# bobhansky/WhittedStyle_Raytracer

Hardware: NVIDIA B200
Metric: Mrays/s (all ray types), out/water_bunny_tex.txt + shadow soft @ 3840x2160 (higher is better)
Workload: dtype f32

## Files before the change

### whittedstyle_raytracer_b200/csrc/cuda/bvh_build.cuh

```cuda
#pragma once
#include <cooperative_groups.h>
#include <cub/device/device_radix_sort.cuh>

#include <cfloat>

#include "ploc_bvh.h"
#include "shaft_cull.h"
#include "wide_bvh.h"
#include "../../../include/wrt_scene.h"

namespace wrt {

#define WRT_PLOC_THREADS 256

enum BuildState { BS_ALLOC = 0, BS_ROOT = 1, BS_DEPTH = 2, BS_PASSES = 3, BS_ERROR = 4, BS_LEAVES = 5, BS_TOTAL = 8 };

struct BuildBuffers {
    PlocTree tree;
    unsigned long long* keys[2];
    int* vals[2];
    int* cl[2];
    int* nn;
    int* blk;
    int* state;
// ... 180 lines not shown
        if (oct & 1) { t = lo.x; lo.x = hi.x; hi.x = t; }
        if (oct & 2) { t = lo.y; lo.y = hi.y; hi.y = t; }
        if (oct & 4) { t = lo.z; lo.z = hi.z; hi.z = t; }
        dst[2 * ((size_t)oct * n_nodes + i)] = lo;
        dst[2 * ((size_t)oct * n_nodes + i) + 1] = hi;
    }
}

__global__ void __launch_bounds__(256) k_wide4_copies(const float4* __restrict__ onodes, int n_nodes, float4* dst) {
    const int pairs = n_nodes / 2;
    const long long total = 8ll * pairs;
    for (long long g = blockIdx.x * (long long)blockDim.x + threadIdx.x; g < total; g += (long long)gridDim.x * blockDim.x) {
        const int oct = (int)(g / pairs);
        const int c = 2 * (int)(g - (long long)oct * pairs);
        if (c == 0) continue;
        float4 out[8];
        wrt_wide4_node(onodes + 2 * (size_t)oct * n_nodes, c, oct, out);
        float4* d = dst + WRT_WIDE_FLOAT4_PER_RECORD * ((size_t)oct * n_nodes + c);
#pragma unroll
        for (int i = 0; i < 8; i++) d[i] = out[i];
    }
}

__global__ void __launch_bounds__(256) k_pack_prims(int n_prims, const float* __restrict__ prim_geom, const unsigned* __restrict__ prim_flags,
                                                    const int* __restrict__ prim_material, const int* __restrict__ prim_texture,
                                                    const int* __restrict__ prim_normalmap, const int* __restrict__ prim_object,
                                                    const float* __restrict__ prim_normals, const float* __restrict__ prim_uv,
                                                    const float* __restrict__ materials, int n_materials, int n_textures, int n_normalmaps,
                                                    float4* geom, float4* attr, int4* ids, float4* tri_aux, int* flags_out) {
    int bad = 0;
    float slack = 0.f;
    for (int p = blockIdx.x * blockDim.x + threadIdx.x; p < n_prims; p += gridDim.x * blockDim.x) {
        const float* g = prim_geom + 12 * (size_t)p;
        const int mat = prim_material[p];
        const unsigned flags = prim_flags[p];
// ... 40 lines not shown
```

### whittedstyle_raytracer_b200/csrc/cuda/dev_traverse.cuh

```cuda
#pragma once
#include "dev_math.cuh"
#include "prune_rule.h"
#include "wide_bvh.h"
#include "shadow_assoc.h"
#include "../../../include/wrt_scene.h"

namespace wrt {

#define WRT_INLINE_LIGHTS 4

struct DevScene {
    const float4* nodes;
    const float4* fnodes;
    const float4* onodes;
    const float4* ronodes;
    const float4* wnodes;
    const float4* dnodes;
    const float4* geom;
    const float4* prim_box;
    const float4* tri_aux;
    const WrtPathCode* path_codes;
    const float4* attr;
    const int4*   ids;
    const int*    object_prim;
// ... 161 lines not shown
        asm volatile("prefetch.global.L1 [%0];" ::"l"(nodes + 2 * far_link));
#endif
        cur = right_first ? linkR : linkL;
        return true;
    }
    if (hl) { cur = linkL; return true; }
    if (hr) { cur = linkR; return true; }
    if (st.empty()) return false;
    cur = st.pop();
    return true;
}

#ifndef WRT_WIDE4
#define WRT_WIDE4 1
#endif
template <bool NEAR_FIRST, class LeafFn>
__device__ __forceinline__ bool traverse_step4(const float4* __restrict__ wnodes, const Ray& r, Stack& st, int& cur,
                                               const float& limit, LeafFn&& leaf) {
    const float4* n = wnodes + WRT_WIDE_FLOAT4_PER_RECORD * (size_t)cur;
    float4 a0, a1, b0, b1, c0, c1, d0, d1;
    ldg8(n, a0, a1);
    ldg8(n + 2, b0, b1);
    ldg8(n + 4, c0, c1);
    ldg8(n + 6, d0, d1);
    float t0, t1, t2, t3;
    bool h0 = slab_presorted(a0, a1, r, t0), h1 = slab_presorted(b0, b1, r, t1);
    bool h2 = slab_presorted(c0, c1, r, t2), h3 = slab_presorted(d0, d1, r, t3);
    int l0 = __float_as_int(a0.w), l1 = __float_as_int(b0.w), l2 = __float_as_int(c0.w), l3 = __float_as_int(d0.w);
    h0 = h0 && !(t0 > limit); h1 = h1 && !(t1 > limit); h2 = h2 && !(t2 > limit); h3 = h3 && !(t3 > limit);
    unsigned leaves = (h0 && l0 < 0 ? 1u : 0u) | (h1 && l1 < 0 ? 2u : 0u) | (h2 && l2 < 0 ? 4u : 0u) | (h3 && l3 < 0 ? 8u : 0u);
    while (leaves) {
        const unsigned j = __ffs(leaves) - 1;
        leaves &= leaves - 1;
        const int lk = j == 0 ? l0 : (j == 1 ? l1 : (j == 2 ? l2 : l3));
        const float tj = j == 0 ? t0 : (j == 1 ? t1 : (j == 2 ? t2 : t3));
        if (!(tj > limit)) leaf(~lk);
    }
    const float inf = INFINITY;
    float k0 = (h0 && l0 >= 0 && !(t0 > limit)) ? t0 : inf, k1 = (h1 && l1 >= 0 && !(t1 > limit)) ? t1 : inf;
    float k2 = (h2 && l2 >= 0 && !(t2 > limit)) ? t2 : inf, k3 = (h3 && l3 >= 0 && !(t3 > limit)) ? t3 : inf;
    if (NEAR_FIRST) {
#define WRT_CSWAP(ka, la, kb, lb) { const bool sw = kb < ka; const float kt = sw ? ka : kb; ka = sw ? kb : ka; kb = kt; const int lt = sw ? la : lb; la = sw ? lb : la; lb = lt; }
        WRT_CSWAP(k0, l0, k1, l1) WRT_CSWAP(k2, l2, k3, l3) WRT_CSWAP(k0, l0, k2, l2) WRT_CSWAP(k1, l1, k3, l3) WRT_CSWAP(k1, l1, k2, l2)
// ... 14 lines not shown
        if (nxt >= 0) { cur = nxt; return true; }
    }
    if (st.empty()) return false;
    cur = st.pop();
    return true;
}

#ifndef WRT_LEAF_DEFER
#define WRT_LEAF_DEFER 2
#endif
#ifndef WRT_LEAF_DEFER_SIMPLE
#define WRT_LEAF_DEFER_SIMPLE 1
#endif
#define WRT_NO_LINK (-2147483647 - 1)
template <bool NEAR_FIRST, class LeafFn>
__device__ __forceinline__ bool traverse_step4_defer(const float4* __restrict__ wnodes, const Ray& r, Stack& st, int& cur,
                                                     const float& limit, LeafFn&& leaf) {
    const float inf = INFINITY;
    int pend = WRT_NO_LINK;
    float tp = -inf;
    if (cur < 0) {
        pend = cur;
        cur = WRT_NO_LINK;
        if (!st.empty()) {
            const int nx = st.pop();
            if (nx >= 0) cur = nx; else ++st.sp;
        }
    }
    if (cur >= 0) {
        const float4* n = wnodes + WRT_WIDE_FLOAT4_PER_RECORD * (size_t)cur;
        float4 a0, a1, b0, b1, c0, c1, d0, d1;
        ldg8(n, a0, a1);
        ldg8(n + 2, b0, b1);
        ldg8(n + 4, c0, c1);
        ldg8(n + 6, d0, d1);
        float t0, t1, t2, t3;
        const bool h0 = slab_presorted(a0, a1, r, t0), h1 = slab_presorted(b0, b1, r, t1);
        const bool h2 = slab_presorted(c0, c1, r, t2), h3 = slab_presorted(d0, d1, r, t3);
        int l0 = __float_as_int(a0.w), l1 = __float_as_int(b0.w), l2 = __float_as_int(c0.w), l3 = __float_as_int(d0.w);
        float k0 = (h0 && !(t0 > limit)) ? t0 : inf, k1 = (h1 && !(t1 > limit)) ? t1 : inf;
        float k2 = (h2 && !(t2 > limit)) ? t2 : inf, k3 = (h3 && !(t3 > limit)) ? t3 : inf;
#define WRT_CSWAP(ka, la, kb, lb) { const bool sw = kb < ka; const float kt = sw ? ka : kb; ka = sw ? kb : ka; kb = kt; const int lt = sw ? la : lb; la = sw ? lb : la; lb = lt; }
        if (NEAR_FIRST) { WRT_CSWAP(k0, l0, k1, l1) WRT_CSWAP(k2, l2, k3, l3) WRT_CSWAP(k0, l0, k2, l2) WRT_CSWAP(k1, l1, k3, l3) WRT_CSWAP(k1, l1, k2, l2) }
#undef WRT_CSWAP
#if WRT_LEAF_DEFER_SIMPLE
        if (NEAR_FIRST) {
            const bool tk = (k0 < inf) && (l0 < 0) && (pend == WRT_NO_LINK);
            if (tk) { pend = l0; tp = k0; }
            const float kc = tk ? k1 : k0;
            const int lc = tk ? l1 : l0;
            cur = kc < inf ? lc : WRT_NO_LINK;
            if (k3 < inf) st.push(l3);
            if (k2 < inf) st.push(l2);
            if (!tk && k1 < inf) st.push(l1);
// ... 39 lines not shown
        limit = FLT_MAX; prune_scale = prune;
    }
    __device__ __forceinline__ void set_ray(const DevScene& s, const Ray& r, float prune_cfg) {
        const float o[3] = {r.o.x, r.o.y, r.o.z}, inv[3] = {r.inv.x, r.inv.y, r.inv.z};
        prune_scale = prune_cfg >= 0.f ? wrt_prune_ray_scale(o, inv, s.prune_slack) : -1.f;
    }
    __device__ __forceinline__ void leaf(const DevScene& s, const Ray& r, int p) {
        PrimHit h; float oma; unsigned fl;
        if (prim_test(s, p, r, h, oma, fl)) {
            if (h.t < best.t || (h.t == best.t && p < best.prim)) {
                best.t = h.t; best.prim = p; best.u = h.u; best.v = h.v;
                if (prune_scale >= 0.f) limit = wrt_prune_limit(h.t, prune_scale);
            }
        }
    }
    __device__ __forceinline__ bool begin(const DevScene& s, const float4* nodes, int root, const Ray& r, int& cur) {
        float te;
        float4 lo = ldg4(nodes + 2 * root), hi = ldg4(nodes + 2 * root + 1);
        if (!slab(lo, hi, r, te)) return false;
        int link = __float_as_int(lo.w);
        if (link < 0) { leaf(s, r, ~link); return false; }
        cur = link;
        return true;
    }
};

__device__ __forceinline__ Closest closest_hit(const DevScene& s, const float4* nodes, int root, const Ray& r, Stack& st,
                                               float prune_rel) {
    ClosestState cs;
    cs.reset(prune_rel);
// ... 44 lines not shown
        int k = i;
        while (k > 0 && prim[idx[k - 1]] > key) { idx[k] = idx[k - 1]; --k; }
        idx[k] = i;
    }
    for (int i = 0; i < n; i++) fs[i] = fac[idx[i]];
    return wrt_tree_product(n, idx, fs, code);
}

__device__ __forceinline__ float shadow_value(const DevScene& s, const ShadowAcc& acc) {
    return acc.needs_tree(s.path_codes) ? shadow_tree_value(acc.prim, acc.fac, acc.code, acc.n) : acc.res;
}

__device__ __forceinline__ void shadow_leaf(const DevScene& s, const Ray& r, float dis, int p, ShadowAcc& acc) {
    PrimHit h; float oma; unsigned fl;
    if (prim_test(s, p, r, h, oma, fl) && h.t < dis && !(fl & WRT_PRIM_LIGHT)) acc.add(p, oma, s.path_codes);
}

__device__ __forceinline__ float shadow_product(const DevScene& s, const float4* nodes, const Ray& r, float dis, Stack& st) {
    ShadowAcc acc;
    acc.reset();
    if (s.n_nodes == 0) return acc.res;
    float te;
    float4 lo = ldg4(nodes), hi = ldg4(nodes + 1);
    if (!slab(lo, hi, r, te)) return acc.res;
    int cur = __float_as_int(lo.w);
    if (cur < 0) { shadow_leaf(s, r, dis, ~cur, acc); return acc.res; }
    st.sp = 0;
    const float never = INFINITY;
    while (acc.res != 0.f && traverse_step<false>(nodes, r, st, cur, never, [&](int p) { shadow_leaf(s, r, dis, p, acc); })) {}
    return shadow_value(s, acc);
// ... 175 lines not shown
```

### whittedstyle_raytracer_b200/csrc/cuda/kernels.cuh

```cuda
#pragma once
#include <cooperative_groups.h>

#include "dev_shade.cuh"
#include "shaft_cull.h"
#include "../../../include/wrt_rng.h"
#include "../../../include/wrt_tiles.h"

#ifdef WRT_MIN_BLOCKS
#define WRT_TRACE_BOUNDS __launch_bounds__(128, WRT_MIN_BLOCKS)
#else
#define WRT_TRACE_BOUNDS __launch_bounds__(128)
#endif
#ifndef WRT_TRACE_DEEP_STEPS
#define WRT_TRACE_DEEP_STEPS 8
#endif
namespace wrt {

#ifdef WRT_DEBUG_BOUNDS
__device__ unsigned g_wrt_bounds_line = 0;
__device__ __forceinline__ bool wrt_bounds_ok(bool ok, unsigned line) {
    if (!ok) atomicCAS(&g_wrt_bounds_line, 0u, line);
    return ok;
}
#define WRT_IN_BOUNDS(idx, cap) wrt_bounds_ok((unsigned long long)(idx) < (unsigned long long)(cap), (unsigned)__LINE__)
// ... 291 lines not shown
        if (ref_tree) prune = -1.f;
        const size_t oct_off = (size_t)ray_octant(r.d) * 2 * (size_t)s.n_nodes;
        nodes = (ref_tree ? s.ronodes : s.onodes) + oct_off;
        cs.set_ray(s, r, prune);
        float te;
        float4 lo = ldg4(nodes), hi = ldg4(nodes + 1);
        if (!slab_presorted(lo, hi, r, te)) return false;
        cur = __float_as_int(lo.w);
        if (cur < 0) { cs.leaf(s, r, ~cur); return false; }
        wide = WRT_WIDE4 && !LEVEL0 && !ref_tree;
        if (wide) nodes = s.wnodes + (WRT_WIDE_FLOAT4_PER_RECORD / 2) * oct_off;
        return true;
    }
    __device__ __forceinline__ bool step(int& cur, Stack& st) {
#if WRT_LEAF_DEFER
        if (WRT_WIDE4 && !LEVEL0 && wide) return traverse_step4_defer<true>(nodes, r, st, cur, cs.limit, [&](int p) { cs.leaf(s, r, p); });
#else
        if (WRT_WIDE4 && !LEVEL0 && wide) return traverse_step4<true>(nodes, r, st, cur, cs.limit, [&](int p) { cs.leaf(s, r, p); });
#endif
        return traverse_step<true, true>(nodes, r, st, cur, cs.limit, [&](int p) { cs.leaf(s, r, p); });
    }
    __device__ __forceinline__ bool finish(int&, Stack&) {
        if (WRT_IN_BOUNDS(idx, fb.cap0 > fb.capd ? fb.cap0 : fb.capd))
            fb.hit[idx] = make_float4(cs.best.t, __int_as_float(cs.best.prim), cs.best.u, cs.best.v);
        return false;
    }
};

template <bool LEVEL0>
__global__ void WRT_TRACE_BOUNDS k_trace_closest(const __grid_constant__ DevScene s, const __grid_constant__ FrameBuffers fb,
                                                 const __grid_constant__ PrimaryGen pg, int level, unsigned n0, int work_slot,
                                                 float prune_rel, int refill) {
    extern __shared__ int smem[];
// ... 67 lines not shown
        const size_t oct_off = (size_t)ray_octant(raydir) * 2 * (size_t)s.n_nodes;
        nodes = (ref_tree ? s.ronodes : s.onodes) + oct_off;
        float te;
        float4 lo = ldg4(nodes), hi = ldg4(nodes + 1);
        if (!slab_presorted(lo, hi, r, te)) return false;
        cur = __float_as_int(lo.w);
        if (cur < 0) { shadow_leaf(s, r, dis, ~cur, acc); return false; }
        wide = WRT_WIDE4 && !ref_tree;
        if (wide) nodes = s.wnodes + (WRT_WIDE_FLOAT4_PER_RECORD / 2) * oct_off;
        return true;
    }
    __device__ __forceinline__ bool step(int& cur, Stack& st) {
        const float never = INFINITY;
        bool more;
#if WRT_LEAF_DEFER >= 2
        if (WRT_WIDE4 && wide) more = traverse_step4_defer<false>(nodes, r, st, cur, never, [&](int p) { shadow_leaf(s, r, dis, p, acc); });
#else
        if (WRT_WIDE4 && wide) more = traverse_step4<false>(nodes, r, st, cur, never, [&](int p) { shadow_leaf(s, r, dis, p, acc); });
#endif
        else more = traverse_step<false, true>(nodes, r, st, cur, never, [&](int p) { shadow_leaf(s, r, dis, p, acc); });
        return more && acc.res != 0.f;
    }
    __device__ __forceinline__ bool finish(int&, Stack&) {
        const float v = shadow_value(s, acc);
        if (WRT_IN_BOUNDS(out, (size_t)fb.n_node_cap * s.n_lights)) fb.coeff[out] = v;
        return false;
    }
};

__global__ void WRT_TRACE_BOUNDS k_shadow_hard(const __grid_constant__ DevScene s, const __grid_constant__ FrameBuffers fb, int q, int work_slot, int refill,
                                               int literal) {
    extern __shared__ int smem[];
    Stack st;
// ... 217 lines not shown
                    if (rc == 1) active = true;
                    else pend = rc;
                }
                head += need < avail ? need : avail;
                __syncwarp();
            }
            if (!__any_sync(0xffffffffu, active)) {
                if (drained && head == tail && !__any_sync(0xffffffffu, pend != -2)) break;
                continue;
            }
        }
#pragma unroll 1
        for (int it = 0; it < 4; it++) {
            if (active) {
#if WRT_WIDE4
                const int rc = wrt_shaft_walk_step4(&sh, &w, st.base, st.stride, stack_rows, mine, WRT_LIST_CAP);
#else
                const int rc = wrt_shaft_walk_step(&sh, &w, st.base, st.stride, stack_rows, mine, WRT_LIST_CAP);
#endif
                if (rc != 1) { active = false; pend = rc < 0 ? -1 : w.n; }
            }
        }
    }
    n_empty = __reduce_add_sync(0xffffffffu, n_empty);
    if (lane == 0 && n_empty) atomicAdd(fb.counters + C_NEMPTY, n_empty);
}
#else
__global__ void __launch_bounds__(128, WRT_LISTS_MIN_BLOCKS) k_soft_lists(const __grid_constant__ DevScene s, const __grid_constant__ FrameBuffers fb, int q,
                                                        int work_slot, int stack_rows, SoftListBuffers lb) {
    extern __shared__ int smem[];
    Stack st;
// ... 118 lines not shown
#endif
                        }
                        if (rc == 1) active = true;
                        else pend = rc;
                    }
                }
                if (!__any_sync(0xffffffffu, active)) {
                    if (next >= chunk && !__any_sync(0xffffffffu, pend != -2)) break;
                    continue;
                }
            }
#pragma unroll 1
            for (int it = 0; it < 4; it++) {
                if (active) {
#if WRT_WIDE4
                    const int rc = wrt_shaft_walk_step4(&sh, &w, st.base, st.stride, stack_rows, mine, WRT_LIST_CAP);
#else
                    const int rc = wrt_shaft_walk_step(&sh, &w, st.base, st.stride, stack_rows, mine, WRT_LIST_CAP);
#endif
                    if (rc != 1) { active = false; pend = rc < 0 ? -1 : w.n; }
                }
            }
        }
        __syncwarp();
    }
    n_empty = __reduce_add_sync(0xffffffffu, n_empty);
    if (lane == 0 && n_empty) atomicAdd(fb.counters + C_NEMPTY, n_empty);
}

#endif

// ... 525 lines not shown
```

### whittedstyle_raytracer_b200/csrc/cuda/shaft_cull.h

```cpp
#ifndef WRT_SHAFT_CULL_H
#define WRT_SHAFT_CULL_H

#include <math.h>

#include "wide_bvh.h"

#ifdef __CUDACC__
#define WRT_SHAFT_HD __host__ __device__ __forceinline__
#else
#include <vector_types.h>
#define WRT_SHAFT_HD static inline
#endif

#if defined(__CUDA_ARCH__)
#define WRT_SHAFT_LD4(p) __ldg(p)
#define WRT_SHAFT_LD8(p, a, b) wrt::ldg8(p, a, b)
#else
#define WRT_SHAFT_LD4(p) (*(p))
#define WRT_SHAFT_LD8(p, a, b) do { (a) = (p)[0]; (b) = (p)[1]; } while (0)
#endif

#define WRT_SHAFT_STACK 48
#define WRT_SHAFT_PAD_REL 1e-5f

// ... 58 lines not shown
    float ly = fminf(ay * sh->ilo[1], ay * sh->ihi[1]), uy = fmaxf(by * sh->ilo[1], by * sh->ihi[1]);
    float lz = fminf(az * sh->ilo[2], az * sh->ihi[2]), uz = fmaxf(bz * sh->ilo[2], bz * sh->ihi[2]);
    if (!(sh->use & 1)) { lx = -INFINITY; ux = INFINITY; }
    if (!(sh->use & 2)) { ly = -INFINITY; uy = INFINITY; }
    if (!(sh->use & 4)) { lz = -INFINITY; uz = INFINITY; }
    float lb = fmaxf(lx, fmaxf(ly, lz)), ub = fminf(ux, fminf(uy, uz));
    return lb <= ub && ub >= 0.f;
}

WRT_SHAFT_HD bool wrt_shaft_may_hit_lb(const WrtShaft* sh, const float4 nearp, const float4 farp, float* lb_out) {
    float ax = nearp.x - sh->o[0], ay = nearp.y - sh->o[1], az = nearp.z - sh->o[2];
    float bx = farp.x - sh->o[0], by = farp.y - sh->o[1], bz = farp.z - sh->o[2];
    float lx = fminf(ax * sh->ilo[0], ax * sh->ihi[0]), ux = fmaxf(bx * sh->ilo[0], bx * sh->ihi[0]);
    float ly = fminf(ay * sh->ilo[1], ay * sh->ihi[1]), uy = fmaxf(by * sh->ilo[1], by * sh->ihi[1]);
    float lz = fminf(az * sh->ilo[2], az * sh->ihi[2]), uz = fmaxf(bz * sh->ilo[2], bz * sh->ihi[2]);
    if (!(sh->use & 1)) { lx = -INFINITY; ux = INFINITY; }
    if (!(sh->use & 2)) { ly = -INFINITY; uy = INFINITY; }
    if (!(sh->use & 4)) { lz = -INFINITY; uz = INFINITY; }
    float lb = fmaxf(lx, fmaxf(ly, lz)), ub = fminf(ux, fminf(uy, uz));
    *lb_out = lb;
    return lb <= ub && ub >= 0.f;
}

typedef struct WrtShaftWalk {
    const float4* nodes;
    int cur, sp, n;
} WrtShaftWalk;

WRT_SHAFT_HD int wrt_shaft_walk_begin(const float4* onodes, int n_nodes, const WrtShaft* sh, WrtShaftWalk* w) {
    w->sp = 0; w->n = 0; w->cur = 0; w->nodes = onodes;
// ... 73 lines not shown
        w.f = r0.w; const int linkR = w.i;
        if ((hl && linkL < 0) || (hr && linkR < 0)) return false;
        if (hl && hr) {
            if (sp == WRT_SHAFT_STACK) return false;
            stack[sp++] = linkR;
            cur = linkL;
        } else if (hl) cur = linkL;
        else if (hr) cur = linkR;
        else {
            if (sp == 0) return true;
            cur = stack[--sp];
        }
    }
}

WRT_SHAFT_HD int wrt_shaft_walk_begin4(const float4* onodes, const float4* wnodes, int n_nodes, const WrtShaft* sh, WrtShaftWalk* w) {
    w->sp = 0; w->n = 0; w->cur = 0; w->nodes = wnodes;
    if (n_nodes <= 0) return 0;
    union { float f; int i; } u;
    u.f = WRT_SHAFT_LD4(onodes + (size_t)sh->octant * 2 * (size_t)n_nodes).w;
    w->cur = u.i;
    w->nodes = wnodes + WRT_WIDE_FLOAT4_PER_RECORD * (size_t)sh->octant * (size_t)n_nodes;
    return w->cur < 0 ? -1 : 1;
}

#ifndef WRT_SHAFT_STEP_BRANCHFREE
#define WRT_SHAFT_STEP_BRANCHFREE 1
#endif
#define WRT_SHAFT_CSWAP(ka, la, kb, lb) { const bool sw_ = (kb) < (ka); const float kt_ = sw_ ? (ka) : (kb); (ka) = sw_ ? (kb) : (ka); (kb) = kt_; \
                                          const int lt_ = sw_ ? (la) : (lb); (la) = sw_ ? (lb) : (la); (lb) = lt_; }

WRT_SHAFT_HD int wrt_shaft_walk_step4(const WrtShaft* sh, WrtShaftWalk* w, int* stack, int stack_stride, int stack_cap,
                                      int* out, int out_cap) {
    const float4* nd = w->nodes + WRT_WIDE_FLOAT4_PER_RECORD * (size_t)w->cur;
    float4 a0, a1, b0, b1, c0, c1, d0, d1;
    WRT_SHAFT_LD8(nd, a0, a1);
    WRT_SHAFT_LD8(nd + 2, b0, b1);
    WRT_SHAFT_LD8(nd + 4, c0, c1);
    WRT_SHAFT_LD8(nd + 6, d0, d1);
    float k0, k1, k2, k3;
    const bool h0 = wrt_shaft_may_hit_lb(sh, a0, a1, &k0), h1 = wrt_shaft_may_hit_lb(sh, b0, b1, &k1);
    const bool h2 = wrt_shaft_may_hit_lb(sh, c0, c1, &k2), h3 = wrt_shaft_may_hit_lb(sh, d0, d1, &k3);
    const float inf = INFINITY;
    if (!h0) k0 = inf;
    if (!h1) k1 = inf;
    if (!h2) k2 = inf;
    if (!h3) k3 = inf;
    union { float f; int i; } u;
    u.f = a0.w; int l0 = u.i;
    u.f = b0.w; int l1 = u.i;
    u.f = c0.w; int l2 = u.i;
    u.f = d0.w; int l3 = u.i;
    WRT_SHAFT_CSWAP(k0, l0, k1, l1) WRT_SHAFT_CSWAP(k2, l2, k3, l3) WRT_SHAFT_CSWAP(k0, l0, k2, l2)
    WRT_SHAFT_CSWAP(k1, l1, k3, l3) WRT_SHAFT_CSWAP(k1, l1, k2, l2)
    int n = w->n;
#if WRT_SHAFT_STEP_BRANCHFREE
    if (n + 4 > out_cap || w->sp + 3 > stack_cap) return -1;
    {
        const bool e0 = k0 < inf && l0 < 0, e1 = k1 < inf && l1 < 0, e2 = k2 < inf && l2 < 0, e3 = k3 < inf && l3 < 0;
        if (e0) out[n] = ~l0;
        n += e0 ? 1 : 0;
        if (e1) out[n] = ~l1;
        n += e1 ? 1 : 0;
        if (e2) out[n] = ~l2;
        n += e2 ? 1 : 0;
        if (e3) out[n] = ~l3;
        n += e3 ? 1 : 0;
// ... 24 lines not shown
    int next = -1;
    if (k3 < inf && l3 >= 0) next = l3;
    if (k2 < inf && l2 >= 0) { if (next >= 0) { if (w->sp == stack_cap) return -1; stack[w->sp * stack_stride] = next; ++w->sp; } next = l2; }
    if (k1 < inf && l1 >= 0) { if (next >= 0) { if (w->sp == stack_cap) return -1; stack[w->sp * stack_stride] = next; ++w->sp; } next = l1; }
    if (k0 < inf && l0 >= 0) { if (next >= 0) { if (w->sp == stack_cap) return -1; stack[w->sp * stack_stride] = next; ++w->sp; } next = l0; }
    if (next >= 0) { w->cur = next; return 1; }
    if (w->sp == 0) return 0;
    --w->sp;
    w->cur = stack[w->sp * stack_stride];
    return 1;
}

WRT_SHAFT_HD int wrt_shaft_candidates4(const float4* onodes, const float4* wnodes, int n_nodes, const WrtShaft* sh, int* stack,
                                       int stack_stride, int stack_cap, int* out, int out_cap) {
    WrtShaftWalk w;
    int rc = wrt_shaft_walk_begin4(onodes, wnodes, n_nodes, sh, &w);
    if (rc <= 0) return rc;
    while ((rc = wrt_shaft_walk_step4(sh, &w, stack, stack_stride, stack_cap, out, out_cap)) == 1) {}
    return rc < 0 ? -1 : w.n;
}

WRT_SHAFT_HD bool wrt_shaft_is_empty4(const float4* onodes, const float4* wnodes, int n_nodes, const float o[3], const float tri[9]) {
    if (n_nodes <= 0) return true;
    WrtShaft sh;
    if (!wrt_shaft_make(o, tri, &sh)) return false;
    union { float f; int i; } u;
    u.f = WRT_SHAFT_LD4(onodes + (size_t)sh.octant * 2 * (size_t)n_nodes).w;
    int cur = u.i;
    if (cur < 0) return false;
    const float4* nodes = wnodes + WRT_WIDE_FLOAT4_PER_RECORD * (size_t)sh.octant * (size_t)n_nodes;
    int stack[WRT_SHAFT_STACK];
    int sp = 0;
    while (true) {
        const float4* nd = nodes + WRT_WIDE_FLOAT4_PER_RECORD * (size_t)cur;
        float4 a0, a1, b0, b1, c0, c1, d0, d1;
        WRT_SHAFT_LD8(nd, a0, a1);
        WRT_SHAFT_LD8(nd + 2, b0, b1);
        WRT_SHAFT_LD8(nd + 4, c0, c1);
        WRT_SHAFT_LD8(nd + 6, d0, d1);
        const bool h0 = wrt_shaft_may_hit(&sh, a0, a1), h1 = wrt_shaft_may_hit(&sh, b0, b1);
        const bool h2 = wrt_shaft_may_hit(&sh, c0, c1), h3 = wrt_shaft_may_hit(&sh, d0, d1);
        u.f = a0.w; const int l0 = u.i;
        u.f = b0.w; const int l1 = u.i;
        u.f = c0.w; const int l2 = u.i;
        u.f = d0.w; const int l3 = u.i;
        if ((h0 && l0 < 0) || (h1 && l1 < 0) || (h2 && l2 < 0) || (h3 && l3 < 0)) return false;
        int next = -1;
        if (h3) next = l3;
        if (h2) { if (next >= 0) { if (sp == WRT_SHAFT_STACK) return false; stack[sp++] = next; } next = l2; }
        if (h1) { if (next >= 0) { if (sp == WRT_SHAFT_STACK) return false; stack[sp++] = next; } next = l1; }
        if (h0) { if (next >= 0) { if (sp == WRT_SHAFT_STACK) return false; stack[sp++] = next; } next = l0; }
        if (next >= 0) { cur = next; continue; }
        if (sp == 0) return true;
        cur = stack[--sp];
    }
}

typedef struct WrtShaftPyramid {
    float o[3];
    float D[4][3];
// ... 115 lines not shown
```

### whittedstyle_raytracer_b200/csrc/cuda/wide_bvh.h

```cpp
#ifndef WRT_WIDE_BVH_H
#define WRT_WIDE_BVH_H

#include <float.h>

#ifdef __CUDACC__
#define WRT_WIDE_HD __host__ __device__ __forceinline__
#else
#include <vector_types.h>
#define WRT_WIDE_HD static inline
#endif

#define WRT_WIDE_FLOAT4_PER_RECORD 4

WRT_WIDE_HD void wrt_wide4_node(const float4* src, int c, int oct, float4* out) {
    union { float f; int i; unsigned u; } w;
    for (int k = 0; k < 2; k++) {
        const float4 lo = src[2 * (size_t)(c + k)], hi = src[2 * (size_t)(c + k) + 1];
        w.f = lo.w;
        if (w.i >= 0) {
            const float4* ch = src + 2 * (size_t)w.i;
            out[4 * k + 0] = ch[0]; out[4 * k + 1] = ch[1];
            out[4 * k + 2] = ch[2]; out[4 * k + 3] = ch[3];
        } else {
            out[4 * k + 0] = lo; out[4 * k + 1] = hi;
            float4 e0, e1;
            e0.x = (oct & 1) ? -FLT_MAX : FLT_MAX; e1.x = -e0.x;
            e0.y = (oct & 2) ? -FLT_MAX : FLT_MAX; e1.y = -e0.y;
            e0.z = (oct & 4) ? -FLT_MAX : FLT_MAX; e1.z = -e0.z;
            w.u = 0x80000000u;
            e0.w = w.f; e1.w = 0.f;
            out[4 * k + 2] = e0; out[4 * k + 3] = e1;
        }
    }
}

#endif
```

### whittedstyle_raytracer_b200/csrc/cuda/wrt_cuda.cu

```cuda
#include <algorithm>
#include <cstdio>
#include <chrono>
#include <cstdlib>
#include <cstring>
#include <condition_variable>
#include <functional>
#include <mutex>
#include <string>
#include <thread>
#include <vector>

#include <cuda_runtime.h>

#include "../../../include/wrt_cuda.h"
#include "fast_bvh.hpp"
#include "kernels.cuh"
#include "bvh_build.cuh"

namespace {

thread_local std::string g_err;

int fail(const std::string& msg) {
    g_err = msg;
// ... 760 lines not shown
    ds.object_prim = (const int*)dptr(7);
    ds.lights = (const WrtLight*)dptr(11);
    ds.textures = (const WrtTexture*)dptr(12);
    ds.normalmaps = (const WrtTexture*)dptr(13);
    ds.texels = (const float*)dptr(14);
    ds.path_codes = parts[15].bytes ? (const WrtPathCode*)dptr(15) : nullptr;

    float4 *geom = nullptr, *attr = nullptr, *mats = nullptr, *pbox = nullptr, *taux = nullptr, *fnodes = nullptr, *dnodes = nullptr, *onodes = nullptr, *ronodes = nullptr, *wnodes = nullptr;
    int4* ids = nullptr;
    int* d_flags = nullptr;
    if (dev_alloc(c, (size_t)np * 48, (void**)&geom) || dev_alloc(c, (size_t)np * 64, (void**)&attr) || dev_alloc(c, (size_t)np * 16, (void**)&ids) ||
        dev_alloc(c, (size_t)s->n_materials * 48, (void**)&mats) || dev_alloc(c, (size_t)np * 32, (void**)&pbox) ||
        dev_alloc(c, (size_t)np * 16, (void**)&taux) ||
        dev_alloc(c, (size_t)nn * 32, (void**)&fnodes) || dev_alloc(c, (size_t)nn * 32, (void**)&dnodes) ||
        dev_alloc(c, (size_t)nn * 32 * 8, (void**)&onodes) || dev_alloc(c, (size_t)nn * 32 * 8, (void**)&ronodes) ||
        dev_alloc(c, (size_t)nn * 64 * 8, (void**)&wnodes) ||
        dev_alloc(c, (wrt::BS_TOTAL + 16) * sizeof(int), (void**)&d_flags))
        return 1;
    int* d_state = d_flags + 8;
    float* d_bounds = (float*)(d_flags + 8 + wrt::BS_TOTAL);
    CK(cudaMemsetAsync(d_flags, 0, (wrt::BS_TOTAL + 8) * sizeof(int), st));
    {
        const float init[8] = {FLT_MAX, FLT_MAX, FLT_MAX, -FLT_MAX, -FLT_MAX, -FLT_MAX, 0.f, 0.f};
        memcpy(c->h_counters + wrt::C_TOTAL + 32, init, sizeof init);
        CK(cudaMemcpyAsync(d_bounds, c->h_counters + wrt::C_TOTAL + 32, sizeof init, cudaMemcpyHostToDevice, st));
    }
    const int wide = c->num_sms * 4;
    if (np > 0) {
        ++c->launches;
        wrt::k_pack_prims<<<std::min(wide, (np + 255) / 256), 256, 0, st>>>(
            np, (const float*)dptr(1), (const unsigned*)dptr(2), (const int*)dptr(3), (const int*)dptr(4), (const int*)dptr(5),
// ... 749 lines not shown
```

Baseline: 7137.

## Compress wide BVH4 nodes to quantized 32-byte records with mirrored-ray traversal

Replaces the 64-byte four-child wide node (full float AABBs per child) with a 32-byte record: a per-node origin, per-axis power-of-two scale exponents, and 8-bit quantized child bounds, built with directed rounding so the boxes stay conservative. Traversal mirrors the ray into the positive octant and decodes the quantized bounds. Leaf hits are then confirmed against the exact primitive box, and the shaft-culling walk applies the same mirroring with an exact leaf check. The aim is to halve node memory traffic and cache footprint, at the cost of decode arithmetic, looser boxes causing extra leaf tests, and an extra prim_box load per confirmed hit.

```diff
diff --git a/whittedstyle_raytracer_b200/csrc/cuda/bvh_build.cuh b/whittedstyle_raytracer_b200/csrc/cuda/bvh_build.cuh
--- a/whittedstyle_raytracer_b200/csrc/cuda/bvh_build.cuh
+++ b/whittedstyle_raytracer_b200/csrc/cuda/bvh_build.cuh
@@ -218,11 +218,11 @@
         const int oct = (int)(g / pairs);
         const int c = 2 * (int)(g - (long long)oct * pairs);
         if (c == 0) continue;
-        float4 out[8];
+        float4 out[4];
         wrt_wide4_node(onodes + 2 * (size_t)oct * n_nodes, c, oct, out);
         float4* d = dst + WRT_WIDE_FLOAT4_PER_RECORD * ((size_t)oct * n_nodes + c);
 #pragma unroll
-        for (int i = 0; i < 8; i++) d[i] = out[i];
+        for (int i = 0; i < 4; i++) d[i] = out[i];
     }
 }
 
diff --git a/whittedstyle_raytracer_b200/csrc/cuda/dev_traverse.cuh b/whittedstyle_raytracer_b200/csrc/cuda/dev_traverse.cuh
--- a/whittedstyle_raytracer_b200/csrc/cuda/dev_traverse.cuh
+++ b/whittedstyle_raytracer_b200/csrc/cuda/dev_traverse.cuh
@@ -199,19 +199,46 @@
 #ifndef WRT_WIDE4
 #define WRT_WIDE4 1
 #endif
+__device__ __forceinline__ Ray mirrored_ray(const Ray& r) {
+    Ray m;
+    m.o = mk3(r.d.x < 0 ? -r.o.x : r.o.x, r.d.y < 0 ? -r.o.y : r.o.y, r.d.z < 0 ? -r.o.z : r.o.z);
+    m.d = r.d;
+    m.inv = mk3(fabsf(r.inv.x), fabsf(r.inv.y), fabsf(r.inv.z));
+    return m;
+}
+__device__ __forceinline__ void wide_node_test(const float4* __restrict__ wnodes, int cur, const Ray& rm, bool& h0, bool& h1,
+                                               bool& h2, bool& h3, float& t0, float& t1, float& t2, float& t3, int& l0, int& l1,
+                                               int& l2, int& l3) {
+    const float4* n = wnodes + WRT_WIDE_FLOAT4_PER_RECORD * (size_t)cur;
+    float4 h, lk, qa, qb;
+    ldg8(n, h, lk);
+    ldg8(n + 2, qa, qb);
+    const float sx = wrt_wide_step(h.w, 0), sy = wrt_wide_step(h.w, 1), sz = wrt_wide_step(h.w, 2);
+    float bx0, bx1, by0, by1, bz0, bz1;
+    wrt_wide_rel(h.x, sx, rm.o.x, &bx0, &bx1);
+    wrt_wide_rel(h.y, sy, rm.o.y, &by0, &by1);
+    wrt_wide_rel(h.z, sz, rm.o.z, &bz0, &bz1);
+#define WRT_WIDE_SLAB(j, hj, tj)                                                                                   \
+    {                                                                                                              \
+        const float ax = wrt_wide_near_rel(qa.x, j, sx, bx0) * rm.inv.x, bx = wrt_wide_far_rel(qa.y, j, sx, bx1) * rm.inv.x; \
+        const float ay = wrt_wide_near_rel(qa.z, j, sy, by0) * rm.inv.y, by = wrt_wide_far_rel(qa.w, j, sy, by1) * rm.inv.y; \
+        const float az = wrt_wide_near_rel(qb.x, j, sz, bz0) * rm.inv.z, bz = wrt_wide_far_rel(qb.y, j, sz, bz1) * rm.inv.z; \
+        tj = fmaxf(ax, fmaxf(ay, az));                                                                             \
+        const float tx = fminf(bx, fminf(by, bz));                                                                 \
+        hj = (tj <= tx) && (tx >= 0);                                                                              \
+    }
+    WRT_WIDE_SLAB(0, h0, t0) WRT_WIDE_SLAB(1, h1, t1) WRT_WIDE_SLAB(2, h2, t2) WRT_WIDE_SLAB(3, h3, t3)
+#undef WRT_WIDE_SLAB
+    l0 = __float_as_int(lk.x); l1 = __float_as_int(lk.y); l2 = __float_as_int(lk.z); l3 = __float_as_int(lk.w);
+    h0 = h0 && l0 != WRT_WIDE_EMPTY; h1 = h1 && l1 != WRT_WIDE_EMPTY; h2 = h2 && l2 != WRT_WIDE_EMPTY; h3 = h3 && l3 != WRT_WIDE_EMPTY;
+}
 template <bool NEAR_FIRST, class LeafFn>
-__device__ __forceinline__ bool traverse_step4(const float4* __restrict__ wnodes, const Ray& r, Stack& st, int& cur,
+__device__ __forceinline__ bool traverse_step4(const float4* __restrict__ wnodes, const Ray& rm, Stack& st, int& cur,
                                                const float& limit, LeafFn&& leaf) {
-    const float4* n = wnodes + WRT_WIDE_FLOAT4_PER_RECORD * (size_t)cur;
-    float4 a0, a1, b0, b1, c0, c1, d0, d1;
-    ldg8(n, a0, a1);
-    ldg8(n + 2, b0, b1);
-    ldg8(n + 4, c0, c1);
-    ldg8(n + 6, d0, d1);
     float t0, t1, t2, t3;
-    bool h0 = slab_presorted(a0, a1, r, t0), h1 = slab_presorted(b0, b1, r, t1);
-    bool h2 = slab_presorted(c0, c1, r, t2), h3 = slab_presorted(d0, d1, r, t3);
-    int l0 = __float_as_int(a0.w), l1 = __float_as_int(b0.w), l2 = __float_as_int(c0.w), l3 = __float_as_int(d0.w);
+    bool h0, h1, h2, h3;
+    int l0, l1, l2, l3;
+    wide_node_test(wnodes, cur, rm, h0, h1, h2, h3, t0, t1, t2, t3, l0, l1, l2, l3);
     h0 = h0 && !(t0 > limit); h1 = h1 && !(t1 > limit); h2 = h2 && !(t2 > limit); h3 = h3 && !(t3 > limit);
     unsigned leaves = (h0 && l0 < 0 ? 1u : 0u) | (h1 && l1 < 0 ? 2u : 0u) | (h2 && l2 < 0 ? 4u : 0u) | (h3 && l3 < 0 ? 8u : 0u);
     while (leaves) {
@@ -256,7 +283,7 @@
 #endif
 #define WRT_NO_LINK (-2147483647 - 1)
 template <bool NEAR_FIRST, class LeafFn>
-__device__ __forceinline__ bool traverse_step4_defer(const float4* __restrict__ wnodes, const Ray& r, Stack& st, int& cur,
+__device__ __forceinline__ bool traverse_step4_defer(const float4* __restrict__ wnodes, const Ray& rm, Stack& st, int& cur,
                                                      const float& limit, LeafFn&& leaf) {
     const float inf = INFINITY;
     int pend = WRT_NO_LINK;
@@ -270,16 +297,10 @@
         }
     }
     if (cur >= 0) {
-        const float4* n = wnodes + WRT_WIDE_FLOAT4_PER_RECORD * (size_t)cur;
-        float4 a0, a1, b0, b1, c0, c1, d0, d1;
-        ldg8(n, a0, a1);
-        ldg8(n + 2, b0, b1);
-        ldg8(n + 4, c0, c1);
-        ldg8(n + 6, d0, d1);
         float t0, t1, t2, t3;
-        const bool h0 = slab_presorted(a0, a1, r, t0), h1 = slab_presorted(b0, b1, r, t1);
-        const bool h2 = slab_presorted(c0, c1, r, t2), h3 = slab_presorted(d0, d1, r, t3);
-        int l0 = __float_as_int(a0.w), l1 = __float_as_int(b0.w), l2 = __float_as_int(c0.w), l3 = __float_as_int(d0.w);
+        bool h0, h1, h2, h3;
+        int l0, l1, l2, l3;
+        wide_node_test(wnodes, cur, rm, h0, h1, h2, h3, t0, t1, t2, t3, l0, l1, l2, l3);
         float k0 = (h0 && !(t0 > limit)) ? t0 : inf, k1 = (h1 && !(t1 > limit)) ? t1 : inf;
         float k2 = (h2 && !(t2 > limit)) ? t2 : inf, k3 = (h3 && !(t3 > limit)) ? t3 : inf;
 #define WRT_CSWAP(ka, la, kb, lb) { const bool sw = kb < ka; const float kt = sw ? ka : kb; ka = sw ? kb : ka; kb = kt; const int lt = sw ? la : lb; la = sw ? lb : la; lb = lt; }
@@ -349,6 +370,19 @@
             }
         }
     }
+    __device__ __forceinline__ void leaf_confirm(const DevScene& s, const Ray& r, int p) {
+        PrimHit h; float oma; unsigned fl;
+        if (prim_test(s, p, r, h, oma, fl)) {
+            if (h.t < best.t || (h.t == best.t && p < best.prim)) {
+                float te;
+                float4 blo, bhi;
+                ldg8(s.prim_box + 2 * (size_t)p, blo, bhi);
+                if (!slab(blo, bhi, r, te)) return;
+                best.t = h.t; best.prim = p; best.u = h.u; best.v = h.v;
+                if (prune_scale >= 0.f) limit = wrt_prune_limit(h.t, prune_scale);
+            }
+        }
+    }
     __device__ __forceinline__ bool begin(const DevScene& s, const float4* nodes, int root, const Ray& r, int& cur) {
         float te;
         float4 lo = ldg4(nodes + 2 * root), hi = ldg4(nodes + 2 * root + 1);
@@ -423,6 +457,16 @@
 __device__ __forceinline__ void shadow_leaf(const DevScene& s, const Ray& r, float dis, int p, ShadowAcc& acc) {
     PrimHit h; float oma; unsigned fl;
     if (prim_test(s, p, r, h, oma, fl) && h.t < dis && !(fl & WRT_PRIM_LIGHT)) acc.add(p, oma, s.path_codes);
+}
+
+__device__ __forceinline__ void shadow_leaf_confirm(const DevScene& s, const Ray& r, float dis, int p, ShadowAcc& acc) {
+    PrimHit h; float oma; unsigned fl;
+    if (prim_test(s, p, r, h, oma, fl) && h.t < dis && !(fl & WRT_PRIM_LIGHT)) {
+        float te;
+        float4 blo, bhi;
+        ldg8(s.prim_box + 2 * (size_t)p, blo, bhi);
+        if (slab(blo, bhi, r, te)) acc.add(p, oma, s.path_codes);
+    }
 }
 
 __device__ __forceinline__ float shadow_product(const DevScene& s, const float4* nodes, const Ray& r, float dis, Stack& st) {
diff --git a/whittedstyle_raytracer_b200/csrc/cuda/kernels.cuh b/whittedstyle_raytracer_b200/csrc/cuda/kernels.cuh
--- a/whittedstyle_raytracer_b200/csrc/cuda/kernels.cuh
+++ b/whittedstyle_raytracer_b200/csrc/cuda/kernels.cuh
@@ -329,9 +329,9 @@
     }
     __device__ __forceinline__ bool step(int& cur, Stack& st) {
 #if WRT_LEAF_DEFER
-        if (WRT_WIDE4 && !LEVEL0 && wide) return traverse_step4_defer<true>(nodes, r, st, cur, cs.limit, [&](int p) { cs.leaf(s, r, p); });
+        if (WRT_WIDE4 && !LEVEL0 && wide) return traverse_step4_defer<true>(nodes, mirrored_ray(r), st, cur, cs.limit, [&](int p) { cs.leaf_confirm(s, r, p); });
 #else
-        if (WRT_WIDE4 && !LEVEL0 && wide) return traverse_step4<true>(nodes, r, st, cur, cs.limit, [&](int p) { cs.leaf(s, r, p); });
+        if (WRT_WIDE4 && !LEVEL0 && wide) return traverse_step4<true>(nodes, mirrored_ray(r), st, cur, cs.limit, [&](int p) { cs.leaf_confirm(s, r, p); });
 #endif
         return traverse_step<true, true>(nodes, r, st, cur, cs.limit, [&](int p) { cs.leaf(s, r, p); });
     }
@@ -429,9 +429,9 @@
         const float never = INFINITY;
         bool more;
 #if WRT_LEAF_DEFER >= 2
-        if (WRT_WIDE4 && wide) more = traverse_step4_defer<false>(nodes, r, st, cur, never, [&](int p) { shadow_leaf(s, r, dis, p, acc); });
+        if (WRT_WIDE4 && wide) more = traverse_step4_defer<false>(nodes, mirrored_ray(r), st, cur, never, [&](int p) { shadow_leaf_confirm(s, r, dis, p, acc); });
 #else
-        if (WRT_WIDE4 && wide) more = traverse_step4<false>(nodes, r, st, cur, never, [&](int p) { shadow_leaf(s, r, dis, p, acc); });
+        if (WRT_WIDE4 && wide) more = traverse_step4<false>(nodes, mirrored_ray(r), st, cur, never, [&](int p) { shadow_leaf_confirm(s, r, dis, p, acc); });
 #endif
         else more = traverse_step<false, true>(nodes, r, st, cur, never, [&](int p) { shadow_leaf(s, r, dis, p, acc); });
         return more && acc.res != 0.f;
@@ -679,7 +679,7 @@
         for (int it = 0; it < 4; it++) {
             if (active) {
 #if WRT_WIDE4
-                const int rc = wrt_shaft_walk_step4(&sh, &w, st.base, st.stride, stack_rows, mine, WRT_LIST_CAP);
+                const int rc = wrt_shaft_walk_step4(&sh, &w, s.onodes, s.wnodes, st.base, st.stride, stack_rows, mine, WRT_LIST_CAP);
 #else
                 const int rc = wrt_shaft_walk_step(&sh, &w, st.base, st.stride, stack_rows, mine, WRT_LIST_CAP);
 #endif
@@ -828,7 +828,7 @@
             for (int it = 0; it < 4; it++) {
                 if (active) {
 #if WRT_WIDE4
-                    const int rc = wrt_shaft_walk_step4(&sh, &w, st.base, st.stride, stack_rows, mine, WRT_LIST_CAP);
+                    const int rc = wrt_shaft_walk_step4(&sh, &w, s.onodes, s.wnodes, st.base, st.stride, stack_rows, mine, WRT_LIST_CAP);
 #else
                     const int rc = wrt_shaft_walk_step(&sh, &w, st.base, st.stride, stack_rows, mine, WRT_LIST_CAP);
 #endif
diff --git a/whittedstyle_raytracer_b200/csrc/cuda/shaft_cull.h b/whittedstyle_raytracer_b200/csrc/cuda/shaft_cull.h
--- a/whittedstyle_raytracer_b200/csrc/cuda/shaft_cull.h
+++ b/whittedstyle_raytracer_b200/csrc/cuda/shaft_cull.h
@@ -96,6 +96,18 @@
     float lx = fminf(ax * sh->ilo[0], ax * sh->ihi[0]), ux = fmaxf(bx * sh->ilo[0], bx * sh->ihi[0]);
     float ly = fminf(ay * sh->ilo[1], ay * sh->ihi[1]), uy = fmaxf(by * sh->ilo[1], by * sh->ihi[1]);
     float lz = fminf(az * sh->ilo[2], az * sh->ihi[2]), uz = fmaxf(bz * sh->ilo[2], bz * sh->ihi[2]);
+    if (!(sh->use & 1)) { lx = -INFINITY; ux = INFINITY; }
+    if (!(sh->use & 2)) { ly = -INFINITY; uy = INFINITY; }
+    if (!(sh->use & 4)) { lz = -INFINITY; uz = INFINITY; }
+    float lb = fmaxf(lx, fmaxf(ly, lz)), ub = fminf(ux, fminf(uy, uz));
+    *lb_out = lb;
+    return lb <= ub && ub >= 0.f;
+}
+
+WRT_SHAFT_HD bool wrt_shaft_may_hit_rel(const WrtShaft* sh, const float a[3], const float b[3], float* lb_out) {
+    float lx = fminf(a[0] * sh->ilo[0], a[0] * sh->ihi[0]), ux = fmaxf(b[0] * sh->ilo[0], b[0] * sh->ihi[0]);
+    float ly = fminf(a[1] * sh->ilo[1], a[1] * sh->ihi[1]), uy = fmaxf(b[1] * sh->ilo[1], b[1] * sh->ihi[1]);
+    float lz = fminf(a[2] * sh->ilo[2], a[2] * sh->ihi[2]), uz = fmaxf(b[2] * sh->ilo[2], b[2] * sh->ihi[2]);
     if (!(sh->use & 1)) { lx = -INFINITY; ux = INFINITY; }
     if (!(sh->use & 2)) { ly = -INFINITY; uy = INFINITY; }
     if (!(sh->use & 4)) { lz = -INFINITY; uz = INFINITY; }
@@ -199,14 +211,56 @@
     }
 }
 
-WRT_SHAFT_HD int wrt_shaft_walk_begin4(const float4* onodes, const float4* wnodes, int n_nodes, const WrtShaft* sh, WrtShaftWalk* w) {
+WRT_SHAFT_HD void wrt_shaft_mirror(WrtShaft* sh) {
+    for (int k = 0; k < 3; k++) {
+        if (!((sh->octant >> k) & 1)) continue;
+        const float a = sh->ilo[k], b = sh->ihi[k];
+        sh->o[k] = -sh->o[k]; sh->ilo[k] = -b; sh->ihi[k] = -a;
+    }
+}
+
+WRT_SHAFT_HD bool wrt_shaft_leaf_exact(const WrtShaft* msh, const float4* orecs, int rec) {
+    float4 a, b;
+    WRT_SHAFT_LD8(orecs + 2 * (size_t)rec, a, b);
+    if (msh->octant & 1) { a.x = -a.x; b.x = -b.x; }
+    if (msh->octant & 2) { a.y = -a.y; b.y = -b.y; }
+    if (msh->octant & 4) { a.z = -a.z; b.z = -b.z; }
+    return wrt_shaft_may_hit(msh, a, b);
+}
+
+WRT_SHAFT_HD int wrt_shaft_walk_begin4(const float4* onodes, const float4* wnodes, int n_nodes, WrtShaft* sh, WrtShaftWalk* w) {
     w->sp = 0; w->n = 0; w->cur = 0; w->nodes = wnodes;
     if (n_nodes <= 0) return 0;
     union { float f; int i; } u;
     u.f = WRT_SHAFT_LD4(onodes + (size_t)sh->octant * 2 * (size_t)n_nodes).w;
     w->cur = u.i;
     w->nodes = wnodes + WRT_WIDE_FLOAT4_PER_RECORD * (size_t)sh->octant * (size_t)n_nodes;
+    wrt_shaft_mirror(sh);
     return w->cur < 0 ? -1 : 1;
+}
+
+WRT_SHAFT_HD void wrt_shaft_wide_node(const WrtShaft* msh, const float4* nd, const float4* orecs, bool* h, float* k, int* l) {
+    float4 hd, lk, qa, qb;
+    WRT_SHAFT_LD8(nd, hd, lk);
+    WRT_SHAFT_LD8(nd + 2, qa, qb);
+    const float sx = wrt_wide_step(hd.w, 0), sy = wrt_wide_step(hd.w, 1), sz = wrt_wide_step(hd.w, 2);
+    float bx0, bx1, by0, by1, bz0, bz1;
+    wrt_wide_rel(hd.x, sx, msh->o[0], &bx0, &bx1);
+    wrt_wide_rel(hd.y, sy, msh->o[1], &by0, &by1);
+    wrt_wide_rel(hd.z, sz, msh->o[2], &bz0, &bz1);
+    union { float f; int i; } u;
+    u.f = lk.x; l[0] = u.i;
+    u.f = lk.y; l[1] = u.i;
+    u.f = lk.z; l[2] = u.i;
+    u.f = lk.w; l[3] = u.i;
+    u.f = qb.z; const int rec0 = u.i;
+    u.f = qb.w; const int rec2 = u.i;
+    for (int j = 0; j < 4; j++) {
+        const float a[3] = {wrt_wide_near_rel(qa.x, j, sx, bx0), wrt_wide_near_rel(qa.z, j, sy, by0), wrt_wide_near_rel(qb.x, j, sz, bz0)};
+        const float b[3] = {wrt_wide_far_rel(qa.y, j, sx, bx1), wrt_wide_far_rel(qa.w, j, sy, by1), wrt_wide_far_rel(qb.y, j, sz, bz1)};
+        h[j] = wrt_shaft_may_hit_rel(msh, a, b, &k[j]) && l[j] != WRT_WIDE_EMPTY;
+        if (h[j] && l[j] < 0) h[j] = wrt_shaft_leaf_exact(msh, orecs, (j < 2 ? rec0 : rec2) + (j & 1));
+    }
 }
 
 #ifndef WRT_SHAFT_STEP_BRANCHFREE
@@ -215,27 +269,20 @@
 #define WRT_SHAFT_CSWAP(ka, la, kb, lb) { const bool sw_ = (kb) < (ka); const float kt_ = sw_ ? (ka) : (kb); (ka) = sw_ ? (kb) : (ka); (kb) = kt_; \
                                           const int lt_ = sw_ ? (la) : (lb); (la) = sw_ ? (lb) : (la); (lb) = lt_; }
 
-WRT_SHAFT_HD int wrt_shaft_walk_step4(const WrtShaft* sh, WrtShaftWalk* w, int* stack, int stack_stride, int stack_cap,
-                                      int* out, int out_cap) {
-    const float4* nd = w->nodes + WRT_WIDE_FLOAT4_PER_RECORD * (size_t)w->cur;
-    float4 a0, a1, b0, b1, c0, c1, d0, d1;
-    WRT_SHAFT_LD8(nd, a0, a1);
-    WRT_SHAFT_LD8(nd + 2, b0, b1);
-    WRT_SHAFT_LD8(nd + 4, c0, c1);
-    WRT_SHAFT_LD8(nd + 6, d0, d1);
-    float k0, k1, k2, k3;
-    const bool h0 = wrt_shaft_may_hit_lb(sh, a0, a1, &k0), h1 = wrt_shaft_may_hit_lb(sh, b0, b1, &k1);
-    const bool h2 = wrt_shaft_may_hit_lb(sh, c0, c1, &k2), h3 = wrt_shaft_may_hit_lb(sh, d0, d1, &k3);
+WRT_SHAFT_HD int wrt_shaft_walk_step4(const WrtShaft* sh, WrtShaftWalk* w, const float4* onodes, const float4* wnodes, int* stack,
+                                      int stack_stride, int stack_cap, int* out, int out_cap) {
+    bool hh[4];
+    float kk[4];
+    int ll[4];
+    wrt_shaft_wide_node(sh, w->nodes + WRT_WIDE_FLOAT4_PER_RECORD * (size_t)w->cur, onodes + (w->nodes - wnodes), hh, kk, ll);
+    const bool h0 = hh[0], h1 = hh[1], h2 = hh[2], h3 = hh[3];
+    float k0 = kk[0], k1 = kk[1], k2 = kk[2], k3 = kk[3];
     const float inf = INFINITY;
     if (!h0) k0 = inf;
     if (!h1) k1 = inf;
     if (!h2) k2 = inf;
     if (!h3) k3 = inf;
-    union { float f; int i; } u;
-    u.f = a0.w; int l0 = u.i;
-    u.f = b0.w; int l1 = u.i;
-    u.f = c0.w; int l2 = u.i;
-    u.f = d0.w; int l3 = u.i;
+    int l0 = ll[0], l1 = ll[1], l2 = ll[2], l3 = ll[3];
     WRT_SHAFT_CSWAP(k0, l0, k1, l1) WRT_SHAFT_CSWAP(k2, l2, k3, l3) WRT_SHAFT_CSWAP(k0, l0, k2, l2)
     WRT_SHAFT_CSWAP(k1, l1, k3, l3) WRT_SHAFT_CSWAP(k1, l1, k2, l2)
     int n = w->n;
@@ -290,9 +337,10 @@
 WRT_SHAFT_HD int wrt_shaft_candidates4(const float4* onodes, const float4* wnodes, int n_nodes, const WrtShaft* sh, int* stack,
                                        int stack_stride, int stack_cap, int* out, int out_cap) {
     WrtShaftWalk w;
-    int rc = wrt_shaft_walk_begin4(onodes, wnodes, n_nodes, sh, &w);
+    WrtShaft msh = *sh;
+    int rc = wrt_shaft_walk_begin4(onodes, wnodes, n_nodes, &msh, &w);
     if (rc <= 0) return rc;
-    while ((rc = wrt_shaft_walk_step4(sh, &w, stack, stack_stride, stack_cap, out, out_cap)) == 1) {}
+    while ((rc = wrt_shaft_walk_step4(&msh, &w, onodes, wnodes, stack, stack_stride, stack_cap, out, out_cap)) == 1) {}
     return rc < 0 ? -1 : w.n;
 }
 
@@ -305,21 +353,17 @@
     int cur = u.i;
     if (cur < 0) return false;
     const float4* nodes = wnodes + WRT_WIDE_FLOAT4_PER_RECORD * (size_t)sh.octant * (size_t)n_nodes;
+    const float4* orecs = onodes + (size_t)sh.octant * 2 * (size_t)n_nodes;
+    wrt_shaft_mirror(&sh);
     int stack[WRT_SHAFT_STACK];
     int sp = 0;
     while (true) {
-        const float4* nd = nodes + WRT_WIDE_FLOAT4_PER_RECORD * (size_t)cur;
-        float4 a0, a1, b0, b1, c0, c1, d0, d1;
-        WRT_SHAFT_LD8(nd, a0, a1);
-        WRT_SHAFT_LD8(nd + 2, b0, b1);
-        WRT_SHAFT_LD8(nd + 4, c0, c1);
-        WRT_SHAFT_LD8(nd + 6, d0, d1);
-        const bool h0 = wrt_shaft_may_hit(&sh, a0, a1), h1 = wrt_shaft_may_hit(&sh, b0, b1);
-        const bool h2 = wrt_shaft_may_hit(&sh, c0, c1), h3 = wrt_shaft_may_hit(&sh, d0, d1);
-        u.f = a0.w; const int l0 = u.i;
-        u.f = b0.w; const int l1 = u.i;
-        u.f = c0.w; const int l2 = u.i;
-        u.f = d0.w; const int l3 = u.i;
+        bool h[4];
+        float k[4];
+        int l[4];
+        wrt_shaft_wide_node(&sh, nodes + WRT_WIDE_FLOAT4_PER_RECORD * (size_t)cur, orecs, h, k, l);
+        const bool h0 = h[0], h1 = h[1], h2 = h[2], h3 = h[3];
+        const int l0 = l[0], l1 = l[1], l2 = l[2], l3 = l[3];
         if ((h0 && l0 < 0) || (h1 && l1 < 0) || (h2 && l2 < 0) || (h3 && l3 < 0)) return false;
         int next = -1;
         if (h3) next = l3;
diff --git a/whittedstyle_raytracer_b200/csrc/cuda/wide_bvh.h b/whittedstyle_raytracer_b200/csrc/cuda/wide_bvh.h
--- a/whittedstyle_raytracer_b200/csrc/cuda/wide_bvh.h
+++ b/whittedstyle_raytracer_b200/csrc/cuda/wide_bvh.h
@@ -2,6 +2,8 @@
 #define WRT_WIDE_BVH_H
 
 #include <float.h>
+#include <math.h>
+#include <string.h>
 
 #ifdef __CUDACC__
 #define WRT_WIDE_HD __host__ __device__ __forceinline__
@@ -10,27 +12,127 @@
 #define WRT_WIDE_HD static inline
 #endif
 
-#define WRT_WIDE_FLOAT4_PER_RECORD 4
+#define WRT_WIDE_FLOAT4_PER_RECORD 2
+#define WRT_WIDE_EMPTY (-2147483647 - 1)
+
+#if defined(__CUDA_ARCH__)
+WRT_WIDE_HD float wrt_wide_fma_rd(float a, float b, float c) { return __fmaf_rd(a, b, c); }
+WRT_WIDE_HD float wrt_wide_fma_ru(float a, float b, float c) { return __fmaf_ru(a, b, c); }
+WRT_WIDE_HD float wrt_wide_add_rd(float a, float b) { return __fadd_rd(a, b); }
+WRT_WIDE_HD float wrt_wide_add_ru(float a, float b) { return __fadd_ru(a, b); }
+#else
+static inline float wrt_wide_fma_dir(float a, float b, float c, int up) {
+    const double x = (double)c, y = (double)a * (double)b;
+    const double d = x + y;
+    const double yy = d - x, e = (x - (d - yy)) + (y - yy);
+    float f = (float)d;
+    if (f != f) return f;
+    if (up) { if ((double)f < d || ((double)f == d && e > 0)) f = nextafterf(f, INFINITY); }
+    else    { if ((double)f > d || ((double)f == d && e < 0)) f = nextafterf(f, -INFINITY); }
+    return f;
+}
+WRT_WIDE_HD float wrt_wide_fma_rd(float a, float b, float c) { return wrt_wide_fma_dir(a, b, c, 0); }
+WRT_WIDE_HD float wrt_wide_fma_ru(float a, float b, float c) { return wrt_wide_fma_dir(a, b, c, 1); }
+WRT_WIDE_HD float wrt_wide_add_rd(float a, float b) { return wrt_wide_fma_dir(1.f, a, b, 0); }
+WRT_WIDE_HD float wrt_wide_add_ru(float a, float b) { return wrt_wide_fma_dir(1.f, a, b, 1); }
+#endif
+
+WRT_WIDE_HD float wrt_wide_f(unsigned u) { float f; memcpy(&f, &u, 4); return f; }
+WRT_WIDE_HD unsigned wrt_wide_u(float f) { unsigned u; memcpy(&u, &f, 4); return u; }
+
+WRT_WIDE_HD float wrt_wide_q(float w, int j) {
+#if defined(__CUDA_ARCH__)
+    return __uint_as_float(__byte_perm(__float_as_uint(w), 0x4B000000u, 0x7540u | (unsigned)j));
+#else
+    return 8388608.f + (float)((wrt_wide_u(w) >> (8 * j)) & 0xffu);
+#endif
+}
+WRT_WIDE_HD float wrt_wide_step(float ew, int k) { return wrt_wide_f(((wrt_wide_u(ew) >> (8 * k)) & 0xffu) << 23); }
+
+WRT_WIDE_HD void wrt_wide_rel(float P, float s, float o, float* blo, float* bhi) {
+    *blo = wrt_wide_fma_rd(-8388608.f, s, wrt_wide_add_rd(P, -o));
+    *bhi = wrt_wide_fma_ru(-8388608.f, s, wrt_wide_add_ru(P, -o));
+}
+WRT_WIDE_HD float wrt_wide_near_rel(float qw, int j, float s, float blo) { return wrt_wide_fma_rd(wrt_wide_q(qw, j), s, blo); }
+WRT_WIDE_HD float wrt_wide_far_rel(float qw, int j, float s, float bhi) { return wrt_wide_fma_ru(wrt_wide_q(qw, j), s, bhi); }
+
+WRT_WIDE_HD void wrt_wide_axis(const float* lo, const float* hi, unsigned used, float* P, unsigned* ebyte, unsigned char* qn,
+                               unsigned char* qf) {
+    float mn = INFINITY, mx = -INFINITY;
+    bool finite = true;
+    for (int j = 0; j < 4; j++) {
+        qn[j] = 255; qf[j] = 0;
+        if (!((used >> j) & 1u)) continue;
+        if (!(fabsf(lo[j]) <= FLT_MAX) || !(fabsf(hi[j]) <= FLT_MAX)) { finite = false; continue; }
+        mn = fminf(mn, lo[j]); mx = fmaxf(mx, hi[j]);
+    }
+    if (!finite) {
+        *P = -FLT_MAX; *ebyte = 254;
+        for (int j = 0; j < 4; j++) { qn[j] = 0; qf[j] = 255; }
+        return;
+    }
+    if (!(mn <= mx)) { *P = 0.f; *ebyte = 127; return; }
+    *P = mn;
+    const double ext = (double)mx - (double)mn;
+    int e = 1;
+    while (e < 254 && 255.0 * ldexp(1.0, e - 127) < ext) e++;
+    for (;; e++) {
+        const float s = wrt_wide_f((unsigned)e << 23);
+        bool ok = true;
+        for (int j = 0; j < 4 && ok; j++) {
+            if (!((used >> j) & 1u)) continue;
+            int a = 0, b = 255;
+            while (a < b) { const int m = (a + b + 1) / 2; if (wrt_wide_fma_ru((float)m, s, mn) <= lo[j]) a = m; else b = m - 1; }
+            qn[j] = (unsigned char)a;
+            if (!(wrt_wide_fma_rd(255.f, s, mn) >= hi[j])) { ok = false; break; }
+            a = 0; b = 255;
+            while (a < b) { const int m = (a + b) / 2; if (wrt_wide_fma_rd((float)m, s, mn) >= hi[j]) b = m; else a = m + 1; }
+            qf[j] = (unsigned char)a;
+        }
+        if (ok || e >= 254) { *ebyte = (unsigned)e; return; }
+    }
+}
 
 WRT_WIDE_HD void wrt_wide4_node(const float4* src, int c, int oct, float4* out) {
-    union { float f; int i; unsigned u; } w;
+    int link[4], rec[2];
+    unsigned used = 0;
+    float lo[3][4], hi[3][4];
+    for (int j = 0; j < 4; j++) for (int k = 0; k < 3; k++) { lo[k][j] = 0.f; hi[k][j] = 0.f; }
     for (int k = 0; k < 2; k++) {
-        const float4 lo = src[2 * (size_t)(c + k)], hi = src[2 * (size_t)(c + k) + 1];
-        w.f = lo.w;
-        if (w.i >= 0) {
-            const float4* ch = src + 2 * (size_t)w.i;
-            out[4 * k + 0] = ch[0]; out[4 * k + 1] = ch[1];
-            out[4 * k + 2] = ch[2]; out[4 * k + 3] = ch[3];
-        } else {
-            out[4 * k + 0] = lo; out[4 * k + 1] = hi;
-            float4 e0, e1;
-            e0.x = (oct & 1) ? -FLT_MAX : FLT_MAX; e1.x = -e0.x;
-            e0.y = (oct & 2) ? -FLT_MAX : FLT_MAX; e1.y = -e0.y;
-            e0.z = (oct & 4) ? -FLT_MAX : FLT_MAX; e1.z = -e0.z;
-            w.u = 0x80000000u;
-            e0.w = w.f; e1.w = 0.f;
-            out[4 * k + 2] = e0; out[4 * k + 3] = e1;
+        const float4 r = src[2 * (size_t)(c + k)];
+        const int lk = (int)wrt_wide_u(r.w);
+        rec[k] = lk >= 0 ? lk : c + k;
+        for (int i = 0; i < 2; i++) {
+            const int j = 2 * k + i;
+            if (lk < 0 && i == 1) { link[j] = WRT_WIDE_EMPTY; continue; }
+            const float4 a = src[2 * (size_t)(rec[k] + i)], b = src[2 * (size_t)(rec[k] + i) + 1];
+            link[j] = (int)wrt_wide_u(a.w);
+            used |= 1u << j;
+            const float na[3] = {a.x, a.y, a.z}, fb[3] = {b.x, b.y, b.z};
+            for (int ax = 0; ax < 3; ax++) {
+                const bool m = (oct >> ax) & 1;
+                lo[ax][j] = m ? -na[ax] : na[ax];
+                hi[ax][j] = m ? -fb[ax] : fb[ax];
+            }
         }
+    }
+    float P[3];
+    unsigned eb[3];
+    unsigned char qn[3][4], qf[3][4];
+    for (int ax = 0; ax < 3; ax++) wrt_wide_axis(lo[ax], hi[ax], used, &P[ax], &eb[ax], qn[ax], qf[ax]);
+    unsigned w[16];
+    w[0] = wrt_wide_u(P[0]); w[1] = wrt_wide_u(P[1]); w[2] = wrt_wide_u(P[2]);
+    w[3] = eb[0] | (eb[1] << 8) | (eb[2] << 16);
+    for (int j = 0; j < 4; j++) w[4 + j] = (unsigned)link[j];
+    for (int ax = 0; ax < 3; ax++) {
+        unsigned a = 0, b = 0;
+        for (int j = 0; j < 4; j++) { a |= (unsigned)qn[ax][j] << (8 * j); b |= (unsigned)qf[ax][j] << (8 * j); }
+        w[8 + 2 * ax] = a; w[9 + 2 * ax] = b;
+    }
+    w[14] = (unsigned)rec[0]; w[15] = (unsigned)rec[1];
+    for (int i = 0; i < 4; i++) {
+        out[i].x = wrt_wide_f(w[4 * i]); out[i].y = wrt_wide_f(w[4 * i + 1]);
+        out[i].z = wrt_wide_f(w[4 * i + 2]); out[i].w = wrt_wide_f(w[4 * i + 3]);
     }
 }
 
diff --git a/whittedstyle_raytracer_b200/csrc/cuda/wrt_cuda.cu b/whittedstyle_raytracer_b200/csrc/cuda/wrt_cuda.cu
--- a/whittedstyle_raytracer_b200/csrc/cuda/wrt_cuda.cu
+++ b/whittedstyle_raytracer_b200/csrc/cuda/wrt_cuda.cu
@@ -798,7 +798,7 @@
         dev_alloc(c, (size_t)np * 16, (void**)&taux) ||
         dev_alloc(c, (size_t)nn * 32, (void**)&fnodes) || dev_alloc(c, (size_t)nn * 32, (void**)&dnodes) ||
         dev_alloc(c, (size_t)nn * 32 * 8, (void**)&onodes) || dev_alloc(c, (size_t)nn * 32 * 8, (void**)&ronodes) ||
-        dev_alloc(c, (size_t)nn * 64 * 8, (void**)&wnodes) ||
+        dev_alloc(c, (size_t)nn * 32 * 8, (void**)&wnodes) ||
         dev_alloc(c, (wrt::BS_TOTAL + 16) * sizeof(int), (void**)&d_flags))
         return 1;
     int* d_state = d_flags + 8;
```

Result: slower. 6206, median of 6 (-13.0%).
